# MatthewZhang473/Efficient-Gaussian-Process-on-Graphs

Measured on AMD Instinct MI355X. Metric: GRF kernel-matrices/sec (N=100k graph, m=128 walks; + achieved HBM GB/s of the Gram kernel), higher is better.
Workload: dtype fp64 walk loads, fp32 Phi, exact-product int64 fixed-point Gram, fp32 K

## Files before the change

efficient-gaussian-process-on-graphs_amd/csrc/grf_gram.hip:

```cpp
#include <stdio.h>
#include <stdlib.h>

#include <algorithm>

#include "grf_block.h"

namespace grf {

typedef float f32x4 __attribute__((ext_vector_type(4)));
typedef uint32_t uint4_v __attribute__((ext_vector_type(4)));

#ifndef GRF_GRAM_K_NT
#define GRF_GRAM_K_NT 1
#endif
#if GRF_GRAM_K_NT
#define GRF_K_STORE(v, p) __builtin_nontemporal_store((v), (p))
#define GRF_K_LOAD(p) __builtin_nontemporal_load(p)
#else
#define GRF_K_STORE(v, p) (*(p) = (v))
#define GRF_K_LOAD(p) (*(p))
#endif
#ifndef GRF_GRAM_PIPE_ABLATE
#define GRF_GRAM_PIPE_ABLATE 0
#endif

constexpr int kChunk = 1024;
constexpr int kSub = 8;
constexpr int kPairBytesG = 12;
constexpr int kTripleBytesG = 16;
constexpr int wave_state_bytes(int halves) { return kChunk + halves * 64 * 8; }

__device__ inline long long fx_round(double x) {
    const double magic = 6755399441055744.0;
    const unsigned long long b = (unsigned long long)__double_as_longlong(x + magic);
    const uint32_t hi = (uint32_t)(b >> 32) - 0x43380000u, lo = (uint32_t)b;
    return (long long)(((unsigned long long)hi << 32) | lo);
}

__device__ inline long long fx_fma_round(double a, double v) {
    const double magic = 6755399441055744.0;
    const unsigned long long b = (unsigned long long)__double_as_longlong(__builtin_fma(a, v, magic));
    const uint32_t hi = (uint32_t)(b >> 32) - 0x43380000u, lo = (uint32_t)b;
    return (long long)(((unsigned long long)hi << 32) | lo);
}


__device__ inline int wave_incl_max(int v) {
    v = max(v, __builtin_amdgcn_update_dpp(0, v, 0x111, 0xf, 0xf, false));
    v = max(v, __builtin_amdgcn_update_dpp(0, v, 0x112, 0xf, 0xf, false));
    v = max(v, __builtin_amdgcn_update_dpp(0, v, 0x114, 0xf, 0xf, false));
    v = max(v, __builtin_amdgcn_update_dpp(0, v, 0x118, 0xf, 0xf, false));
    v = max(v, __builtin_amdgcn_update_dpp(0, v, 0x142, 0xa, 0xf, false));
    v = max(v, __builtin_amdgcn_update_dpp(0, v, 0x143, 0xc, 0xf, false));
    return v;
}

template <int NW>
__device__ inline int gram_propagate_ids(unsigned char *bid, int carry, int lane) {
    static_assert(NW == 1 || NW == 2 || NW == 4, "one 4-, 8- or 16-byte LDS access per lane");
    uint32_t w[NW];
    if constexpr (NW == 1) {
        w[0] = reinterpret_cast<uint32_t *>(bid)[lane];
    } else if constexpr (NW == 2) {
        const uint2 x = reinterpret_cast<uint2 *>(bid)[lane];
        w[0] = x.x;
        w[1] = x.y;
    } else {
        const uint4 x = reinterpret_cast<uint4 *>(bid)[lane];
        w[0] = x.x;
        w[1] = x.y;
        w[2] = x.z;
        w[3] = x.w;
    }
    int run = 0;
#pragma unroll
    for (int i = 0; i < NW; ++i) {
        uint32_t o = 0;
#pragma unroll
        for (int b = 0; b < 4; ++b) {
            run = max(run, (int)((w[i] >> (8 * b)) & 0xffu));
            o |= (uint32_t)run << (8 * b);
        }
        w[i] = o;
    }
    int before = __builtin_amdgcn_update_dpp(0, wave_incl_max(run), 0x138, 0xf, 0xf, false);
    before = max(before, carry);
#pragma unroll
    for (int i = 0; i < NW; ++i) {
// ... 37 lines not shown

template <int NW, int TAIL, int kRec>
__device__ __forceinline__ void gram_windows(const GramStream &g, int32_t w0, int32_t c0, int32_t cend, int lane) {
    static_assert(TAIL == 0 || TAIL == 1, "only the last window of a group is ever masked");
    static_assert(kRec == kPairBytesG || kRec == kTripleBytesG, "record pairs or triples");
    const bool last_ok = !TAIL || w0 + (NW - 1) * 64 + lane < cend;
    int m[NW];
#pragma unroll
    for (int u = 0; u < NW; ++u) {
        const int32_t p = w0 + u * 64 + lane;
        m[u] = (u != NW - 1 || last_ok) ? (int)g.st.bid[p - c0] - 1 : 0;
    }
    int32_t pos[NW];
    double sc[NW];
#pragma unroll
    for (int u = 0; u < NW; ++u) {
        pos[u] = g.st.tbase[m[u]] + kRec * (w0 + u * 64 + lane);
        sc[u] = (double)g.st.aval[m[u]] * g.S;
    }
    if (TAIL) {
        pos[NW - 1] = last_ok ? pos[NW - 1] : g.safe;
        sc[NW - 1] = last_ok ? sc[NW - 1] : 0.0;
    }
    __builtin_amdgcn_sched_barrier(0);
    if constexpr (kRec == kTripleBytesG) {
        uint4_v rec[NW];
#pragma unroll
        for (int u = 0; u < NW; ++u) rec[u] = __builtin_amdgcn_raw_buffer_load_b128(g.rec, (uint32_t)pos[u], 0, 0);
        __builtin_amdgcn_sched_barrier(0);
#pragma unroll
        for (int u = 0; u < NW; ++u) {
            const uint32_t cols = rec[u][0], base = cols & 0xe00u;
            uint32_t c[3] = {(cols & 0xfffu) << 3, (base + ((cols >> 12) & 0x3ffu)) << 3, (base + (cols >> 22)) << 3};
#pragma unroll
            for (int q = 0; q < 3; ++q) {
                if (TAIL && u == NW - 1) c[q] = last_ok ? c[q] : (uint32_t)(lane & 15) * 8u;
                const long long v = fx_fma_round(sc[u], (double)__uint_as_float(rec[u][1 + q]));
                __hip_atomic_fetch_add(reinterpret_cast<unsigned long long *>(g.acc + c[q]), (unsigned long long)v,
                                       __ATOMIC_RELAXED, __HIP_MEMORY_SCOPE_WORKGROUP);
            }
        }
        return;
    }
    RecPair rec[NW];
#pragma unroll
    for (int u = 0; u < NW; ++u) {
        const auto v = __builtin_amdgcn_raw_buffer_load_b96(g.rec, (uint32_t)pos[u], 0, 0);
        rec[u].cols = v[0];
        rec[u].v0 = __uint_as_float(v[1]);
        rec[u].v1 = __uint_as_float(v[2]);
    }
    __builtin_amdgcn_sched_barrier(0);
#pragma unroll
    for (int u = 0; u < NW; ++u) {
        const long long q0 = fx_fma_round(sc[u], (double)rec[u].v0);
        const long long q1 = fx_fma_round(sc[u], (double)rec[u].v1);
        uint32_t c0 = rec[u].cols & 0xffffu, c1 = rec[u].cols >> 16;
        if (TAIL && u == NW - 1) {
            c0 = last_ok ? c0 : (uint32_t)(lane & 15) * 8u;
            c1 = last_ok ? c1 : (uint32_t)(lane & 15) * 8u;
        }
        __hip_atomic_fetch_add(reinterpret_cast<unsigned long long *>(g.acc + c0), (unsigned long long)q0,
                               __ATOMIC_RELAXED, __HIP_MEMORY_SCOPE_WORKGROUP);
        __hip_atomic_fetch_add(reinterpret_cast<unsigned long long *>(g.acc + c1), (unsigned long long)q1,
                               __ATOMIC_RELAXED, __HIP_MEMORY_SCOPE_WORKGROUP);
    }
}

__device__ inline float fx_to_float(unsigned long long a, int sh) {
    const int lo = (int)(unsigned)(a & 0xffffffffull);
    const int hi = (int)(a >> 32) - (lo >> 31);
    return ldexpf(fmaf((float)hi, 4294967296.0f, (float)lo), -sh);
}

__device__ __forceinline__ void slot_buckets(uint2 d, int32_t sb, int32_t ovf_base, int32_t *t0, int32_t *cnt) {
    const int32_t inl = min((int32_t)d.x, 2);
    t0[0] = sb + 8;
    cnt[0] = inl;
    t0[1] = ovf_base + kPairBytesG * (int32_t)d.y;
    cnt[1] = (int32_t)d.x - inl;
}

constexpr int kGramUnroll = 8;

template <int kV, int kRec = kPairBytesG>
__device__ __forceinline__ void gram_stream_batch(const GramStream &gs, const int32_t *cnt, const int32_t *t0,
                                                  const float *av, int lane) {
    const GramWaveState &st = gs.st;
    int32_t excl[kV];
    int32_t total = 0;
#pragma unroll
    for (int h = 0; h < kV; ++h) {
        const int32_t inc = wave_inclusive_scan<int32_t>(cnt[h]) + total;
        excl[h] = inc - cnt[h];
        total = __builtin_amdgcn_readlane(inc, 63);
    }
#pragma unroll
    for (int h = 0; h < kV; ++h) {
        st.tbase[h * 64 + lane] = t0[h] - kRec * excl[h];
        st.aval[h * 64 + lane] = av[h];
    }
    int carry = 0;
    const int32_t chunk = total <= 256 ? 256 : total <= 512 ? 512 : kChunk;
    for (int32_t c0 = 0; c0 < total; c0 += chunk) {
        const int32_t cend = (total - c0) < chunk ? total : c0 + chunk;
        if (chunk == 256) reinterpret_cast<uint32_t *>(st.bid)[lane] = 0u;
        else if (chunk == 512) reinterpret_cast<uint2 *>(st.bid)[lane] = make_uint2(0u, 0u);
        else reinterpret_cast<uint4 *>(st.bid)[lane] = make_uint4(0u, 0u, 0u, 0u);
        __builtin_amdgcn_wave_barrier();
#pragma unroll
        for (int h = 0; h < kV; ++h)
            if (cnt[h] > 0 && excl[h] >= c0 && excl[h] < cend)
                st.bid[excl[h] - c0] = (unsigned char)(h * 64 + lane + 1);
        __builtin_amdgcn_wave_barrier();
        carry = chunk == 256   ? gram_propagate_ids<1>(st.bid, carry, lane)
                : chunk == 512 ? gram_propagate_ids<2>(st.bid, carry, lane)
                               : gram_propagate_ids<4>(st.bid, carry, lane);
        __builtin_amdgcn_wave_barrier();
        int32_t w0 = c0;
        for (; w0 + 64 * kGramUnroll <= cend; w0 += 64 * kGramUnroll)
            gram_windows<kGramUnroll, 0, kRec>(gs, w0, c0, cend, lane);
        if (w0 < cend) {
            static_assert(kGramUnroll == 8, "the tail switch lists 1 .. 8 windows");
            switch ((cend - w0 + 63) >> 6) {
                case 1: gram_windows<1, 1, kRec>(gs, w0, c0, cend, lane); break;
                case 2: gram_windows<2, 1, kRec>(gs, w0, c0, cend, lane); break;
                case 3: gram_windows<3, 1, kRec>(gs, w0, c0, cend, lane); break;
                case 4: gram_windows<4, 1, kRec>(gs, w0, c0, cend, lane); break;
                case 5: gram_windows<5, 1, kRec>(gs, w0, c0, cend, lane); break;
                case 6: gram_windows<6, 1, kRec>(gs, w0, c0, cend, lane); break;
                case 7: gram_windows<7, 1, kRec>(gs, w0, c0, cend, lane); break;
                default: gram_windows<8, 1, kRec>(gs, w0, c0, cend, lane); break;
            }
        }
        __builtin_amdgcn_wave_barrier();
    }
}

typedef unsigned long long u64x2 __attribute__((ext_vector_type(2)));

template <bool kZero>
__device__ __forceinline__ void gram_tile_out(unsigned long long *acc, float *krow, bool vec, int64_t c_lo,
                                              int64_t wlen, int sh, bool addk, int tid, int threads) {
#if GRF_GRAM_PIPE_ABLATE == 2
    constexpr bool store = !kZero;
#else
    constexpr bool store = true;
#endif
    u64x2 *acc2 = reinterpret_cast<u64x2 *>(acc);
    const u64x2 z2 = {0ull, 0ull};
    int64_t done = c_lo;
    if (vec) {
        const int64_t n4 = wlen / 4;
        f32x4 *k4 = reinterpret_cast<f32x4 *>(krow);
        for (int64_t i = c_lo / 4 + tid; i < n4; i += threads) {
            const u64x2 a = acc2[2 * i], b = acc2[2 * i + 1];
            f32x4 o;
            o[0] = fx_to_float(a[0], sh);
            o[1] = fx_to_float(a[1], sh);
            o[2] = fx_to_float(b[0], sh);
            o[3] = fx_to_float(b[1], sh);
            if (addk) o += __builtin_nontemporal_load(&k4[i]);
            if (store) GRF_K_STORE(o, &k4[i]);
            if (kZero) {
                acc2[2 * i] = z2;
                acc2[2 * i + 1] = z2;
            }
        }
        done = n4 * 4;
    }
    for (int64_t i = done + tid; i < wlen; i += threads) {
        if (store) krow[i] = addk ? fx_to_float(acc[i], sh) + krow[i] : fx_to_float(acc[i], sh);
        if (kZero) acc[i] = 0ull;
    }
}

constexpr size_t gram_lds_bytes(int64_t W, int waves, int halves) {
    return (size_t)W * 8 + (size_t)waves * wave_state_bytes(halves);
}

struct GramTiles {
    int64_t rows, W, nb;
    bool sym;
    int32_t k_begin, k_end;
    int64_t J_off = 0;
    int64_t t_rows = -1;
    bool add_k = false;
    __host__ __device__ int64_t count(int64_t J) const {
        if (!sym) return rows;
        const int64_t c = (J + 1) * W;
        return c < rows ? c : rows;
    }
    __host__ __device__ int64_t before(int64_t J) const {
        if (!sym) return J * rows;
        const int64_t full = (rows + W - 1) / W - 1;
        return J <= full ? W * J * (J + 1) / 2 : W * full * (full + 1) / 2 + (J - full) * rows;
    }
    __host__ __device__ int64_t total() const { return before(nb); }
    __device__ void locate(int64_t t, int64_t &J, int64_t &r) const {
        if (!sym) {
            J = t / rows;
        } else {
            J = (int64_t)((sqrt(8.0 * (double)(t / W) + 1.0) - 1.0) * 0.5);
            if (J > nb - 1) J = nb - 1;
            while (J > 0 && before(J) > t) --J;
            while (J < nb - 1 && before(J + 1) <= t) ++J;
        }
        r = t - before(J);
    }
};

template <int kWaves, int kHalves, bool kSlot, int kRec>
__global__ __launch_bounds__(64 * kWaves) void gram_sparse_kernel(
    int64_t n_total, int64_t row_begin, GramTiles tl, int64_t t_begin, const int64_t *__restrict__ ptr,
    const int32_t *__restrict__ idx, const float *__restrict__ val, const uint2 *__restrict__ t_desc,
    const unsigned char *__restrict__ t_rec, int32_t unit, const int32_t *__restrict__ rowshift,
    float *__restrict__ K, int64_t ldk, const uint16_t *__restrict__ t_split,
    int64_t ovf_base, int32_t balance, const int32_t *__restrict__ row_cuts) {
    extern __shared__ __attribute__((aligned(16))) unsigned long long acc[];
    static_assert(!kSlot || kHalves == 1, "slot streams: 2 virtual buckets per nonzero, u8 ids <= 128");
    static_assert(!kSlot || kRec == kPairBytesG, "slots hold pairs");
    const int tid = threadIdx.x, lane = tid & 63, wave = tid >> 6;
    const int64_t W = tl.W;
    constexpr int kB = 64 * kHalves;
    constexpr int kV = kSlot ? 2 * kHalves : kHalves;

    int64_t J, r;
    tl.locate(t_begin + (int64_t)blockIdx.x, J, r);
    const int64_t J_local = J;
    J += tl.J_off;
    const int64_t row = row_begin + r;
    const int64_t j0 = J * W;
    const int64_t t_rows = tl.t_rows < 0 ? n_total : tl.t_rows;
    const int64_t wlen = (t_rows - j0) < W ? (t_rows - j0) : W;
    const int64_t e0 = ptr[row], e1 = ptr[row + 1];
    const int64_t boff = J * n_total;
    const int sh = rowshift[row];
    const int32_t line0 = kSlot ? 0 : (int32_t)t_desc[boff].x;
    const unsigned char *brec = t_rec + (int64_t)line0 * unit;
    const int dsub = (t_split && tl.sym && r >= J_local * W) ? (int)(((r - J_local * W) * kSub) / W) : 0;

    u64x2 *acc2 = reinterpret_cast<u64x2 *>(acc);
    const u64x2 z2 = {0ull, 0ull};
    for (int64_t i = tid; i < W / 2; i += 64 * kWaves) acc2[i] = z2;
    if (kWaves > 1) __syncthreads();
    else __builtin_amdgcn_wave_barrier();

    const GramStream gs{gram_wave_state(acc, W, wave, kV),
                        __builtin_amdgcn_make_buffer_rsrc(const_cast<unsigned char *>(brec), (short)0, 0x7fffffff,
                                                          0x00020000),
                        reinterpret_cast<unsigned char *>(acc), ldexp(1.0, sh), kSlot ? 8 : 0};
    const int64_t nnz_row = e1 - e0, share = (nnz_row + kWaves - 1) / kWaves;
    int64_t ws0 = balance ? e0 + (wave * share < nnz_row ? wave * share : nnz_row) : e0 + (int64_t)wave * kB;
    int64_t ws1 = balance ? e0 + ((wave + 1) * share < nnz_row ? (wave + 1) * share : nnz_row) : e1;
    if (row_cuts) {
        static_assert(8 % kWaves == 0, "row cuts: 8 shares per row");
        constexpr int kStep = 8 / kWaves;
        ws0 = e0 + row_cuts[row * 8 + wave * kStep];
        ws1 = wave + 1 < kWaves ? e0 + row_cuts[row * 8 + (wave + 1) * kStep] : e1;
    }
    const int64_t gstep = (balance || row_cuts) ? kB : (int64_t)kB * kWaves;
    for (int64_t g0 = ws0; g0 < ws1; g0 += gstep) {
        const int64_t gend = (balance || row_cuts) ? ((g0 + kB) < ws1 ? g0 + kB : ws1) : e1;
        int32_t cnt[kV], t0[kV];
        float av[kV];
#pragma unroll
        for (int h = 0; h < kHalves; ++h) {
            const int64_t e = g0 + h * 64 + lane;
            int32_t k = e < gend ? idx[e] : -1;
            if (k < tl.k_begin || k >= tl.k_end) k = -1;
            const float a = k >= 0 ? val[e] : 0.f;
            if constexpr (kSlot) {
                const int64_t sb = 32 * (boff + (k >= 0 ? k : 0));
                const uint2 d = k >= 0 ? *reinterpret_cast<const uint2 *>(t_rec + sb) : make_uint2(0u, 0u);
                slot_buckets(d, (int32_t)sb, (int32_t)ovf_base, &t0[2 * h], &cnt[2 * h]);
                av[2 * h] = a;
                av[2 * h + 1] = a;
            } else {
                av[h] = a;
                const uint2 d = k >= 0 ? t_desc[boff + k] : make_uint2((uint32_t)line0, 0u);
                const int32_t skip = (dsub > 0 && k >= 0) ? min((int32_t)(t_split[(boff + k) * kSub + dsub] >> 1), (int32_t)d.y) : 0;
                t0[h] = ((int32_t)d.x - line0) * unit + kRec * skip;
                cnt[h] = (int32_t)d.y - skip;
            }
        }
        gram_stream_batch<kV, kRec>(gs, cnt, t0, av, lane);
    }
    if (kWaves > 1) __syncthreads();
    else __builtin_amdgcn_wave_barrier();

    gram_tile_out<false>(acc, K + r * ldk + j0, (ldk & 3) == 0 && (j0 & 3) == 0, (int64_t)dsub * (W / kSub), wlen, sh,
                         tl.add_k, tid, 64 * kWaves);
}

__device__ __forceinline__ void pipe_barrier() { asm volatile("s_waitcnt lgkmcnt(0)\n\ts_barrier" ::: "memory"); }

struct PipeNz {
    int32_t k;
    float a;
    int32_t sh;
    int32_t nb;
    int64_t ws0;
};

template <int kWv>
__global__ __launch_bounds__(64 * kWv) void gram_slot_pipe_kernel(
    int64_t n_cols, int64_t row_begin, int64_t rows, int64_t W, int64_t t_rows, int64_t n_tiles,
    const int64_t *__restrict__ ptr, const int32_t *__restrict__ idx, const float *__restrict__ val,
    const unsigned char *__restrict__ t_rec, const int32_t *__restrict__ rowshift, float *__restrict__ K,
    int64_t ldk, int64_t ovf_base, int64_t pad_cap, const int32_t *__restrict__ pad_cnt) {
    extern __shared__ __attribute__((aligned(16))) unsigned long long acc[];
    const int tid = threadIdx.x, lane = tid & 63, wave = tid >> 6;
    const int64_t G = gridDim.x;
    const int64_t n_mine = (int64_t)blockIdx.x < n_tiles ? (n_tiles - 1 - (int64_t)blockIdx.x) / G + 1 : 0;
    u64x2 *acc2 = reinterpret_cast<u64x2 *>(acc);
    const u64x2 z2 = {0ull, 0ull};
    for (int64_t q = tid; q < W / 2; q += 64 * kWv) acc2[q] = z2;
    const GramWaveState wst = gram_wave_state(acc, W, wave, 2);
    const __amdgpu_buffer_rsrc_t rec_rs =
        __builtin_amdgcn_make_buffer_rsrc(const_cast<unsigned char *>(t_rec), (short)0, 0x7fffffff, 0x00020000);
    auto tile_row = [&](int64_t i, int64_t &J) -> int64_t {
        const int64_t t = (int64_t)blockIdx.x + i * G;
        J = t / rows;
        return row_begin + (t - J * rows);
    };
    auto load_bounds = [&](int64_t i, int64_t &pv, int32_t &pc, int32_t &shv) {
        if (i >= n_mine) {
            pv = 0;
            pc = 0;
            shv = 0;
            return;
        }
        int64_t J;
        const int64_t row = tile_row(i, J);
        if (pad_cap > 0) {
            const __amdgpu_buffer_rsrc_t rc =
                __builtin_amdgcn_make_buffer_rsrc(const_cast<int32_t *>(pad_cnt + row), (short)0, 4, 0x00020000);
            pc = (int32_t)__builtin_amdgcn_raw_buffer_load_b32(rc, 0u, 0, 0);
        } else {
            const __amdgpu_buffer_rsrc_t rp =
                __builtin_amdgcn_make_buffer_rsrc(const_cast<int64_t *>(ptr + row), (short)0, 16, 0x00020000);
            const auto v = __builtin_amdgcn_raw_buffer_load_b64(rp, (uint32_t)(lane & 1) * 8u, 0, 0);
            pv = (int64_t)(((uint64_t)v[1] << 32) | v[0]);
        }
        const __amdgpu_buffer_rsrc_t rs =
            __builtin_amdgcn_make_buffer_rsrc(const_cast<int32_t *>(rowshift + row), (short)0, 4, 0x00020000);
        shv = (int32_t)__builtin_amdgcn_raw_buffer_load_b32(rs, 0u, 0, 0);
    };
    auto load_nz = [&](int64_t i, int64_t pv, int32_t pc, int32_t shv, PipeNz &z) {
        if (i >= n_mine) {
            z = PipeNz{-1, 0.f, 0, 0, 0};
            return;
        }
        auto lane_i64 = [&](int l) {
            const uint32_t lo = (uint32_t)__builtin_amdgcn_readlane((int)(uint32_t)pv, l);
            const uint32_t hi = (uint32_t)__builtin_amdgcn_readlane((int)(uint32_t)((uint64_t)pv >> 32), l);
            return (int64_t)(((uint64_t)hi << 32) | lo);
        };
        int64_t e0, e1;
        if (pad_cap > 0) {
            int64_t J;
            e0 = tile_row(i, J) * pad_cap;
            e1 = e0 + (int64_t)__builtin_amdgcn_readlane(pc, 0);
        } else {
            e0 = lane_i64(0);
            e1 = lane_i64(1);
        }
        const int64_t nnz = e1 - e0, share = (nnz + kWv - 1) / kWv;
        const int64_t s0 = wave * share < nnz ? wave * share : nnz, s1 = (wave + 1) * share < nnz ? (wave + 1) * share : nnz;
        const int64_t e = e0 + s0 + lane;
        const bool ok = s0 + lane < s1;
        z.k = ok ? idx[e] : -1;
        z.a = ok ? val[e] : 0.f;
        z.sh = shv;
        z.nb = (int32_t)(s1 - s0);
        z.ws0 = e0 + s0;
    };
    auto load_hdr = [&](int64_t i, int32_t k) -> uint2 {
        if (i >= n_mine || k < 0) return make_uint2(0u, 0u);
        int64_t J;
        tile_row(i, J);
        return *reinterpret_cast<const uint2 *>(t_rec + 32 * (J * n_cols + k));
    };
    auto run_batch = [&](const GramStream &gs, int64_t J, int32_t k, float a, uint2 d) {
        int32_t cnt[2], t0[2];
        const float av[2] = {a, a};
        slot_buckets(d, (int32_t)(32 * (J * n_cols + (k >= 0 ? k : 0))), (int32_t)ovf_base, t0, cnt);
        gram_stream_batch<2>(gs, cnt, t0, av, lane);
    };
    int64_t pv = 0;
    int32_t pc = 0, shv;
    PipeNz T0, T1;
    load_bounds(0, pv, pc, shv);
    load_nz(0, pv, pc, shv, T0);
    uint2 d0 = load_hdr(0, T0.k);
    load_bounds(1, pv, pc, shv);
    load_nz(1, pv, pc, shv, T1);
    load_bounds(2, pv, pc, shv);
    __builtin_amdgcn_s_waitcnt(0);
    pipe_barrier();
    for (int64_t i = 0; i < n_mine; ++i) {
        const uint2 d1 = load_hdr(i + 1, T1.k);
        PipeNz T2;
        load_nz(i + 2, pv, pc, shv, T2);
        load_bounds(i + 3, pv, pc, shv);
        int64_t J;
        const int64_t row = tile_row(i, J);
        if (GRF_GRAM_PIPE_ABLATE != 1) {
            const GramStream gs{wst, rec_rs, reinterpret_cast<unsigned char *>(acc), ldexp(1.0, T0.sh), 8};
            run_batch(gs, J, T0.k, T0.a, d0);
            for (int32_t g = 64; g < T0.nb; g += 64) {
                const int64_t e = T0.ws0 + g + lane;
                const bool ok = g + lane < T0.nb;
                const int32_t k = ok ? idx[e] : -1;
                const float a = ok ? val[e] : 0.f;
                const uint2 d = k >= 0 ? *reinterpret_cast<const uint2 *>(t_rec + 32 * (J * n_cols + k)) : make_uint2(0u, 0u);
                run_batch(gs, J, k, a, d);
            }
        }
        __builtin_amdgcn_s_waitcnt(0);
        pipe_barrier();
        const int64_t r = row - row_begin, j0 = J * W;
        const int64_t wlen = (t_rows - j0) < W ? (t_rows - j0) : W;
        gram_tile_out<true>(acc, K + r * ldk + j0, (ldk & 3) == 0 && (j0 & 3) == 0, 0, wlen, T0.sh, false, tid,
                            64 * kWv);
        pipe_barrier();
        T0 = T1;
        d0 = d1;
        T1 = T2;
    }
}

__global__ __launch_bounds__(256) void hub_panel_kernel(int64_t n_rows, const int64_t *__restrict__ ptr,
                                                        const int32_t *__restrict__ idx, const float *__restrict__ val,
                                                        const int32_t *__restrict__ hub_pos, float *__restrict__ P,
                                                        int64_t ldp) {
    const int64_t row = (int64_t)blockIdx.x * 4 + (threadIdx.x >> 6);
    if (row >= n_rows) return;
    const int lane = threadIdx.x & 63;
    const int64_t e1 = ptr[row + 1];
    for (int64_t e = ptr[row] + lane; e < e1; e += 64) {
        const int32_t q = hub_pos[idx[e]];
        if (q >= 0) P[row * ldp + q] = val[e];
    }
}

__global__ __launch_bounds__(256) void transpose_drop_kernel(int64_t n_bands, int64_t n_cols, uint2 *__restrict__ t_desc,
                                                             const int32_t *__restrict__ cols, int32_t n_drop) {
    const int64_t t = (int64_t)blockIdx.x * 256 + threadIdx.x;
    if (t >= n_bands * n_drop) return;
    const int64_t J = t / n_drop;
    t_desc[J * n_cols + cols[t - J * n_drop]].y = 0u;
}

__device__ __forceinline__ void gram_mirror_tri_coords(int64_t nt, int64_t b, int64_t &bi_out, int64_t &bj_out) {
    int64_t bi = (int64_t)(((double)(2 * nt + 1) - sqrt((double)(2 * nt + 1) * (double)(2 * nt + 1) - 8.0 * (double)b)) * 0.5);
    auto first = [nt](int64_t i) { return i * nt - i * (i - 1) / 2; };
    if (bi < 0) bi = 0;
    if (bi > nt - 1) bi = nt - 1;
    while (bi > 0 && first(bi) > b) --bi;
    while (bi < nt - 1 && first(bi + 1) <= b) ++bi;
    bi_out = bi;
    bj_out = bi + (b - first(bi));
}

__device__ __forceinline__ void gram_mirror_block_at(int64_t n, int64_t bi, int64_t bj, float *__restrict__ K,
                                                     int64_t ldk, float (*tile)[65]) {
    const int64_t i0 = bi * 64, j0 = bj * 64;
    const int t = threadIdx.x;
    const bool full = i0 + 64 <= n && j0 + 64 <= n && (ldk & 3) == 0;
#pragma unroll
    for (int q = 0; q < 4; ++q) {
        const int y = (t >> 4) + 16 * q, x = (t & 15) * 4;
        const int64_t i = i0 + y;
        if (full) {
            const f32x4 v = __builtin_nontemporal_load(reinterpret_cast<const f32x4 *>(K + i * ldk + j0 + x));
            tile[y][x] = v[0]; tile[y][x + 1] = v[1]; tile[y][x + 2] = v[2]; tile[y][x + 3] = v[3];
        } else {
#pragma unroll
            for (int c = 0; c < 4; ++c) tile[y][x + c] = (i < n && j0 + x + c < n) ? K[i * ldk + j0 + x + c] : 0.f;
        }
    }
    __syncthreads();
#pragma unroll
    for (int q = 0; q < 4; ++q) {
        const int y = (t >> 4) + 16 * q, x = (t & 15) * 4;
        const int64_t j = j0 + y;
        if (full && bi != bj) {
            f32x4 v;
            v[0] = tile[x][y]; v[1] = tile[x + 1][y]; v[2] = tile[x + 2][y]; v[3] = tile[x + 3][y];
            __builtin_nontemporal_store(v, reinterpret_cast<f32x4 *>(K + j * ldk + i0 + x));
        } else {
#pragma unroll
            for (int c = 0; c < 4; ++c) {
                const int64_t i = i0 + x + c;
                if (j < n && i < n && j > i) K[j * ldk + i] = tile[x + c][y];
            }
        }
    }
}

__device__ __forceinline__ void gram_mirror_block_swz_at(int64_t n, int64_t bi, int64_t bj, float *__restrict__ K,
                                                         int64_t ldk, float *__restrict__ tile) {
    const int64_t i0 = bi * 64, j0 = bj * 64;
    const int t = threadIdx.x;
    const bool full = i0 + 64 <= n && j0 + 64 <= n && (ldk & 3) == 0 && bi != bj;
    if (!full) {
// ... 71 lines not shown
}

}

using namespace grf;

extern "C" {
#pragma GCC visibility push(default)

size_t grf_gram_workspace_bytes(void) { return 256; }

struct GramArgs {
    int64_t n_total;
    int64_t row_begin;
    const int64_t *ptr;
    const int32_t *idx;
    const float *val;
    int64_t pad_cap;
    const int32_t *pad_cnt;
    int32_t unit;
    int32_t rec_kind;
    const uint32_t *t_desc;
    const void *t_rec;
    const void *t_split;
    const int32_t *rowshift;
    const int32_t *row_cuts;
    float *K;
    int64_t ldk;
    hipStream_t st;
};

static int32_t gram_check(const char *fn, bool args_ok, int32_t unit, const void *t_rec, int64_t ldk, int64_t ld_min,
                          int64_t band_width) {
    GRF_REQUIRE(args_ok, GRF_EINVAL, "%s: bad arguments", fn);
    GRF_REQUIRE(unit == GRF_REC_LINE || unit == GRF_REC_PACKED || unit == GRF_REC_SLOT, GRF_EINVAL,
                "%s: rec_unit must be GRF_REC_LINE, GRF_REC_PACKED or GRF_REC_SLOT", fn);
    GRF_REQUIRE(((uintptr_t)t_rec & 127) == 0, GRF_EINVAL, "%s: t_rec must be 128-byte aligned", fn);
    GRF_REQUIRE(ldk >= ld_min, GRF_EINVAL, "%s: ldk < %lld columns", fn, (long long)ld_min);
    GRF_REQUIRE(band_width >= 64 && band_width % 64 == 0 && band_width <= 8192, GRF_EUNSUPPORTED,
                "%s: band_width must be a multiple of 64 in [64, 8192]", fn);
    return GRF_OK;
}

static int32_t gram_tiles_launch(const GramArgs &a, const GramTiles &tl, int64_t t_first, int64_t t_last) {
    const bool slot = a.unit == GRF_REC_SLOT;
    GRF_REQUIRE(a.rec_kind == GRF_REC_PAIRS ||
                    (a.rec_kind == GRF_REC_TRIPLES && a.unit == GRF_REC_LINE && tl.W <= 4096 && !a.t_split),
                GRF_EINVAL, "gram: GRF_REC_TRIPLES needs line buckets, band_width <= 4096 and no t_split");
    const unsigned char *rec = reinterpret_cast<const unsigned char *>(a.t_rec);
    const int64_t ovf_base = slot ? 32 * tl.nb * a.n_total : 0;
    if (slot) {
        GRF_REQUIRE(!a.t_split, GRF_EUNSUPPORTED, "gram: GRF_REC_SLOT has no split variant");
        GRF_REQUIRE(ovf_base < ((int64_t)1 << 30), GRF_EUNSUPPORTED,
                    "gram: GRF_REC_SLOT slots beyond 32-bit record offsets");
        const bool pipe = [] {
            const char *e = getenv("GRF_GRAM_PIPE");
            return !e || atoi(e) != 0;
        }();
        const bool pipe_ok = !tl.sym && tl.t_rows >= 0 && !tl.add_k && tl.k_begin == 0 &&
                             tl.k_end == (int32_t)a.n_total && t_first == 0 && t_last == tl.total() && tl.J_off == 0;
        GRF_REQUIRE(a.pad_cap == 0 || pipe_ok, GRF_EUNSUPPORTED,
                    "gram: padded rows need the pipelined column-block kernel (a whole non-symmetric launch)");
        if ((pipe || a.pad_cap > 0) && pipe_ok) {
            const size_t lds = gram_lds_bytes(tl.W, 8, 2);
            int dev = 0, n_cu = 0;
            GRF_CHECK_HIP(hipGetDevice(&dev));
            GRF_CHECK_HIP(hipDeviceGetAttribute(&n_cu, hipDeviceAttributeMultiprocessorCount, dev));
            const int per_cu = (int)std::max<int64_t>(1, (int64_t)(160 * 1024) / (int64_t)lds);
            const int64_t grid = std::min<int64_t>((int64_t)std::max(n_cu, 1) * per_cu, t_last);
            gram_slot_pipe_kernel<8><<<(unsigned)grid, 512, lds, a.st>>>(
                a.n_total, a.row_begin, tl.rows, tl.W, tl.t_rows, t_last, a.ptr, a.idx, a.val, rec, a.rowshift, a.K,
                a.ldk, ovf_base, a.pad_cap, a.pad_cnt);
            GRF_CHECK_LAUNCH("gram_slot_pipe_kernel");
            return GRF_OK;
        }
    }
    const uint16_t *split = tl.sym ? (const uint16_t *)a.t_split : nullptr;
    const int waves = (slot || tl.W > 4096) ? 8 : 4;
    const size_t lds = gram_lds_bytes(tl.W, waves, (slot || waves == 4) ? 2 : 1);
    const int32_t balance = (slot || tl.t_rows < 0) ? 1 : 0;
    const int64_t max_tiles = ((1ll << 32) - 1) / (64 * waves);
    for (int64_t t0 = t_first; t0 < t_last; t0 += max_tiles) {
        const int64_t nt = (t_last - t0) < max_tiles ? (t_last - t0) : max_tiles;
#define GRF_GRAM_LAUNCH(WV, H, SLOT, REC)                                                                         \
    gram_sparse_kernel<WV, H, SLOT, REC><<<(unsigned)nt, 64 * WV, lds, a.st>>>(                                   \
        a.n_total, a.row_begin, tl, t0, a.ptr, a.idx, a.val, reinterpret_cast<const uint2 *>(a.t_desc), rec, a.unit, \
        a.rowshift, a.K, a.ldk, split, ovf_base, balance, a.row_cuts)
        if (slot) GRF_GRAM_LAUNCH(8, 1, true, kPairBytesG);
        else if (waves == 8) GRF_GRAM_LAUNCH(8, 1, false, kPairBytesG);
        else if (a.rec_kind == GRF_REC_TRIPLES) GRF_GRAM_LAUNCH(4, 2, false, kTripleBytesG);
        else GRF_GRAM_LAUNCH(4, 2, false, kPairBytesG);
#undef GRF_GRAM_LAUNCH
        GRF_CHECK_LAUNCH("gram_sparse_kernel");
    }
    return GRF_OK;
}

static int32_t gram_sparse_rows_impl(const char *fn, int32_t rec_kind, int64_t n_total, int64_t row_begin, int64_t row_end,
                                     int64_t k_begin, int64_t k_end, const int64_t *ptr, const int32_t *idx,
                                     const float *val, int64_t band_width, int32_t rec_unit, const uint32_t *t_desc,
                                     const void *t_rec, const int32_t *t_rowshift, float *K, int64_t ldk,
                                     grf_stream_t stream) {
    int32_t rc = gram_check(fn,
                            n_total >= 0 && 0 <= row_begin && row_begin <= row_end && row_end <= n_total && ptr &&
                                t_desc && K && t_rowshift && t_rec,
                            rec_unit, t_rec, ldk, n_total, band_width);
    if (rc != GRF_OK) return rc;
    GRF_REQUIRE(0 <= k_begin && k_begin <= k_end && k_end <= n_total, GRF_EINVAL, "%s: bad column slice [%lld, %lld)",
                fn, (long long)k_begin, (long long)k_end);
    if (row_end == row_begin || n_total == 0) return GRF_OK;
    const GramTiles tl{row_end - row_begin, band_width, cdiv<int64_t>(n_total, band_width), false, (int32_t)k_begin,
                       (int32_t)k_end};
    const GramArgs a{n_total,  row_begin, ptr,    idx,   val,     0,          nullptr,
                     rec_unit, rec_kind,  t_desc, t_rec, nullptr, t_rowshift, nullptr, K, ldk, S(stream)};
    return gram_tiles_launch(a, tl, 0, tl.total());
}

int32_t grf_gram_sparse(int64_t n_total, int64_t row_begin, int64_t row_end, const int64_t *ptr, const int32_t *idx,
                        const float *val, int64_t band_width, int32_t rec_unit, const uint32_t *t_desc,
                        const void *t_rec, const int32_t *t_rowshift, float *K, int64_t ldk, void *workspace,
                        size_t workspace_bytes, grf_stream_t stream) {
    return gram_sparse_rows_impl("grf_gram_sparse", GRF_REC_PAIRS, n_total, row_begin, row_end, 0, n_total, ptr, idx, val,
                                 band_width, rec_unit, t_desc, t_rec, t_rowshift, K, ldk, stream);
}

int32_t grf_gram_sparse_rec(int32_t rec_kind, int64_t n_total, int64_t row_begin, int64_t row_end, const int64_t *ptr,
                            const int32_t *idx, const float *val, int64_t band_width, int32_t rec_unit,
                            const uint32_t *t_desc, const void *t_rec, const int32_t *t_rowshift, float *K, int64_t ldk,
                            grf_stream_t stream) {
    return gram_sparse_rows_impl("grf_gram_sparse_rec", rec_kind, n_total, row_begin, row_end, 0, n_total, ptr, idx, val,
                                 band_width, rec_unit, t_desc, t_rec, t_rowshift, K, ldk, stream);
}

static int32_t gram_sparse_upper_impl(const char *fn, int32_t rec_kind, int64_t n_total, const int64_t *ptr, const int32_t *idx,
                                      const float *val, int64_t band_width, int32_t rec_unit, const uint32_t *t_desc,
                                      const void *t_rec, const void *t_split, const int32_t *t_rowshift,
                                      const int32_t *row_cuts, float *K, int64_t ldk, int32_t part_begin,
                                      int32_t part_end, int32_t n_parts, bool add_k, grf_stream_t stream) {
    int32_t rc = gram_check(fn, n_total >= 0 && ptr && t_desc && K && t_rowshift && t_rec, rec_unit, t_rec, ldk,
                            n_total, band_width);
    if (rc != GRF_OK) return rc;
    GRF_REQUIRE(n_parts >= 1 && 0 <= part_begin && part_begin <= part_end && part_end <= n_parts, GRF_EINVAL,
                "%s: bad tile parts [%d, %d) of %d", fn, part_begin, part_end, n_parts);
    if (n_total == 0 || part_begin == part_end) return GRF_OK;
    GramTiles tl{n_total, band_width, cdiv<int64_t>(n_total, band_width), true, 0, (int32_t)n_total};
    tl.add_k = add_k;
    const int64_t total = tl.total();
    const int64_t t0 = total * part_begin / n_parts, t1 = total * part_end / n_parts;
    if (t1 <= t0) return GRF_OK;
    GRF_REQUIRE(!row_cuts || rec_unit != GRF_REC_SLOT, GRF_EUNSUPPORTED, "%s: row cuts with slot buckets", fn);
    const GramArgs a{n_total,  0,        ptr,    idx,   val,     0,          nullptr,
                     rec_unit, rec_kind, t_desc, t_rec, t_split, t_rowshift, row_cuts, K, ldk, S(stream)};
    return gram_tiles_launch(a, tl, t0, t1);
}

int32_t grf_gram_sparse_sym(int64_t n_total, const int64_t *ptr, const int32_t *idx, const float *val,
                            int64_t band_width, int32_t rec_unit, const uint32_t *t_desc, const void *t_rec,
                            const void *t_split, const int32_t *t_rowshift, float *K, int64_t ldk, void *workspace, size_t workspace_bytes,
                            grf_stream_t stream) {
    int32_t rc = gram_sparse_upper_impl("grf_gram_sparse_sym", GRF_REC_PAIRS, n_total, ptr, idx, val, band_width, rec_unit, t_desc,
                                        t_rec, t_split, t_rowshift, nullptr, K, ldk, 0, 1, 1, false, stream);
    if (rc != GRF_OK || n_total == 0) return rc;
    return grf_gram_mirror(n_total, K, ldk, 0, stream);
}

int32_t grf_gram_sparse_upper_ex(int64_t n_total, const int64_t *ptr, const int32_t *idx, const float *val,
                                 int64_t band_width, int32_t rec_unit, const uint32_t *t_desc, const void *t_rec,
                                 const void *t_split, const int32_t *t_rowshift, const int32_t *row_cuts, float *K,
                                 int64_t ldk, int32_t part_begin, int32_t part_end, int32_t n_parts, int32_t add_k,
                                 grf_stream_t stream) {
    return gram_sparse_upper_impl("grf_gram_sparse_upper_ex", GRF_REC_PAIRS, n_total, ptr, idx, val, band_width, rec_unit, t_desc,
                                  t_rec, t_split, t_rowshift, row_cuts, K, ldk, part_begin, part_end, n_parts,
                                  add_k != 0, stream);
}
// ... 222 lines not shown
```

Measured before the change: 45.73.

## Add specialised plain symmetric Gram tile path with 32-bit tile indexing

Adds a specialised kernel path for the common full symmetric Gram case without splits, row cuts or accumulate. It locates tiles with 32-bit reciprocal division and a float sqrt, splits each row's nonzeros evenly across waves, and prefetches the next batch of bucket descriptors during streaming. It uses a smaller window unroll of 4 and 32-bit loop indices in the tile output, aiming to cut integer and address overhead and register pressure. It adds a second kernel instantiation, and the float-sqrt locate depends on its correction step to stay exact.

```diff
diff --git a/efficient-gaussian-process-on-graphs_amd/csrc/grf_gram.hip b/efficient-gaussian-process-on-graphs_amd/csrc/grf_gram.hip
--- a/efficient-gaussian-process-on-graphs_amd/csrc/grf_gram.hip
+++ b/efficient-gaussian-process-on-graphs_amd/csrc/grf_gram.hip
@@ -4,6 +4,7 @@
 #include <algorithm>
 
 #include "grf_block.h"
+#include "grf_gram_tiles.h"
 
 namespace grf {
 
@@ -207,8 +208,21 @@
 }
 
 constexpr int kGramUnroll = 8;
-
-template <int kV, int kRec = kPairBytesG>
+constexpr int kPlainUnroll = 4;
+
+template <int N, int kRec>
+__device__ __forceinline__ void gram_tail_group(const GramStream &gs, int nw, int32_t w0, int32_t c0, int32_t cend,
+                                                int lane) {
+    if constexpr (N > 1) {
+        if (nw < N) {
+            gram_tail_group<N - 1, kRec>(gs, nw, w0, c0, cend, lane);
+            return;
+        }
+    }
+    gram_windows<N, 1, kRec>(gs, w0, c0, cend, lane);
+}
+
+template <int kV, int kRec = kPairBytesG, int kU = kGramUnroll>
 __device__ __forceinline__ void gram_stream_batch(const GramStream &gs, const int32_t *cnt, const int32_t *t0,
                                                   const float *av, int lane) {
     const GramWaveState &st = gs.st;
@@ -243,21 +257,9 @@
                                : gram_propagate_ids<4>(st.bid, carry, lane);
         __builtin_amdgcn_wave_barrier();
         int32_t w0 = c0;
-        for (; w0 + 64 * kGramUnroll <= cend; w0 += 64 * kGramUnroll)
-            gram_windows<kGramUnroll, 0, kRec>(gs, w0, c0, cend, lane);
-        if (w0 < cend) {
-            static_assert(kGramUnroll == 8, "the tail switch lists 1 .. 8 windows");
-            switch ((cend - w0 + 63) >> 6) {
-                case 1: gram_windows<1, 1, kRec>(gs, w0, c0, cend, lane); break;
-                case 2: gram_windows<2, 1, kRec>(gs, w0, c0, cend, lane); break;
-                case 3: gram_windows<3, 1, kRec>(gs, w0, c0, cend, lane); break;
-                case 4: gram_windows<4, 1, kRec>(gs, w0, c0, cend, lane); break;
-                case 5: gram_windows<5, 1, kRec>(gs, w0, c0, cend, lane); break;
-                case 6: gram_windows<6, 1, kRec>(gs, w0, c0, cend, lane); break;
-                case 7: gram_windows<7, 1, kRec>(gs, w0, c0, cend, lane); break;
-                default: gram_windows<8, 1, kRec>(gs, w0, c0, cend, lane); break;
-            }
-        }
+        for (; w0 + 64 * kU <= cend; w0 += 64 * kU)
+            gram_windows<kU, 0, kRec>(gs, w0, c0, cend, lane);
+        if (w0 < cend) gram_tail_group<kU, kRec>(gs, (cend - w0 + 63) >> 6, w0, c0, cend, lane);
         __builtin_amdgcn_wave_barrier();
     }
 }
@@ -265,8 +267,8 @@
 typedef unsigned long long u64x2 __attribute__((ext_vector_type(2)));
 
 template <bool kZero>
-__device__ __forceinline__ void gram_tile_out(unsigned long long *acc, float *krow, bool vec, int64_t c_lo,
-                                              int64_t wlen, int sh, bool addk, int tid, int threads) {
+__device__ __forceinline__ void gram_tile_out(unsigned long long *acc, float *krow, bool vec, int32_t c_lo,
+                                              int32_t wlen, int sh, bool addk, int tid, int threads) {
 #if GRF_GRAM_PIPE_ABLATE == 2
     constexpr bool store = !kZero;
 #else
@@ -274,11 +276,11 @@
 #endif
     u64x2 *acc2 = reinterpret_cast<u64x2 *>(acc);
     const u64x2 z2 = {0ull, 0ull};
-    int64_t done = c_lo;
+    int32_t done = c_lo;
     if (vec) {
-        const int64_t n4 = wlen / 4;
+        const int32_t n4 = wlen / 4;
         f32x4 *k4 = reinterpret_cast<f32x4 *>(krow);
-        for (int64_t i = c_lo / 4 + tid; i < n4; i += threads) {
+        for (int32_t i = c_lo / 4 + tid; i < n4; i += threads) {
             const u64x2 a = acc2[2 * i], b = acc2[2 * i + 1];
             f32x4 o;
             o[0] = fx_to_float(a[0], sh);
@@ -294,7 +296,7 @@
         }
         done = n4 * 4;
     }
-    for (int64_t i = done + tid; i < wlen; i += threads) {
+    for (int32_t i = done + tid; i < wlen; i += threads) {
         if (store) krow[i] = addk ? fx_to_float(acc[i], sh) + krow[i] : fx_to_float(acc[i], sh);
         if (kZero) acc[i] = 0ull;
     }
@@ -304,40 +306,75 @@
     return (size_t)W * 8 + (size_t)waves * wave_state_bytes(halves);
 }
 
-struct GramTiles {
-    int64_t rows, W, nb;
-    bool sym;
-    int32_t k_begin, k_end;
-    int64_t J_off = 0;
-    int64_t t_rows = -1;
-    bool add_k = false;
-    __host__ __device__ int64_t count(int64_t J) const {
-        if (!sym) return rows;
-        const int64_t c = (J + 1) * W;
-        return c < rows ? c : rows;
-    }
-    __host__ __device__ int64_t before(int64_t J) const {
-        if (!sym) return J * rows;
-        const int64_t full = (rows + W - 1) / W - 1;
-        return J <= full ? W * J * (J + 1) / 2 : W * full * (full + 1) / 2 + (J - full) * rows;
-    }
-    __host__ __device__ int64_t total() const { return before(nb); }
-    __device__ void locate(int64_t t, int64_t &J, int64_t &r) const {
-        if (!sym) {
-            J = t / rows;
-        } else {
-            J = (int64_t)((sqrt(8.0 * (double)(t / W) + 1.0) - 1.0) * 0.5);
-            if (J > nb - 1) J = nb - 1;
-            while (J > 0 && before(J) > t) --J;
-            while (J < nb - 1 && before(J + 1) <= t) ++J;
-        }
-        r = t - before(J);
-    }
-};
-
-template <int kWaves, int kHalves, bool kSlot, int kRec>
+__device__ __forceinline__ void pipe_barrier() { asm volatile("s_waitcnt lgkmcnt(0)\n\ts_barrier" ::: "memory"); }
+
+template <int kWaves, int kHalves, int kRec>
+__device__ __forceinline__ void gram_plain_tile(unsigned long long *acc, uint32_t n_total, const GramTiles32 &t32,
+                                                uint32_t t, const int64_t *__restrict__ ptr,
+                                                const int32_t *__restrict__ idx, const float *__restrict__ val,
+                                                const uint2 *__restrict__ t_desc,
+                                                const unsigned char *__restrict__ t_rec, int32_t unit,
+                                                const int32_t *__restrict__ rowshift, float *__restrict__ K,
+                                                int64_t ldk) {
+    static_assert(kWaves > 1, "the plain tile synchronises its waves with s_barrier");
+    const int tid = threadIdx.x, lane = tid & 63, wave = __builtin_amdgcn_readfirstlane(tid >> 6);
+    constexpr int kB = 64 * kHalves;
+    uint32_t J, r;
+    t32.locate(t, J, r);
+    J += t32.J_off;
+    const uint32_t W = t32.W, j0 = J * W;
+    const int32_t wlen = (int32_t)((n_total - j0) < W ? (n_total - j0) : W);
+    const uint2 *bdesc = t_desc + (uint64_t)J * n_total;
+    const int64_t e0 = ptr[r], e1 = ptr[r + 1];
+    const int sh = rowshift[r];
+    const int32_t line0 = (int32_t)bdesc[0].x;
+    const int32_t *ridx = idx + e0;
+    const float *rval = val + e0;
+    const int32_t nnz_row = (int32_t)(e1 - e0), share = (nnz_row + kWaves - 1) / kWaves;
+    const int32_t s0 = min(wave * share, nnz_row), s1 = min((wave + 1) * share, nnz_row);
+
+    int32_t k[kHalves];
+    float av[kHalves];
+    uint2 d[kHalves];
+    auto load_batch = [&](int32_t g) {
+        const int32_t gend = min(g + kB, s1);
+#pragma unroll
+        for (int h = 0; h < kHalves; ++h) {
+            const int32_t e = g + h * 64 + lane;
+            k[h] = e < gend ? ridx[e] : -1;
+            av[h] = e < gend ? rval[e] : 0.f;
+        }
+#pragma unroll
+        for (int h = 0; h < kHalves; ++h) d[h] = k[h] >= 0 ? bdesc[k[h]] : make_uint2((uint32_t)line0, 0u);
+    };
+    load_batch(s0);
+    u64x2 *acc2 = reinterpret_cast<u64x2 *>(acc);
+    const u64x2 z2 = {0ull, 0ull};
+    for (int32_t i = tid; i < (int32_t)(W / 2); i += 64 * kWaves) acc2[i] = z2;
+    const GramStream gs{gram_wave_state(acc, W, wave, kHalves),
+                        __builtin_amdgcn_make_buffer_rsrc(const_cast<unsigned char *>(t_rec + (int64_t)line0 * unit),
+                                                          (short)0, 0x7fffffff, 0x00020000),
+                        reinterpret_cast<unsigned char *>(acc), ldexp(1.0, sh), 0};
+    pipe_barrier();
+    for (int32_t g = s0; g < s1;) {
+        int32_t cnt[kHalves], t0[kHalves];
+#pragma unroll
+        for (int h = 0; h < kHalves; ++h) {
+            t0[h] = ((int32_t)d[h].x - line0) * unit;
+            cnt[h] = (int32_t)d[h].y;
+        }
+        gram_stream_batch<kHalves, kRec, kPlainUnroll>(gs, cnt, t0, av, lane);
+        g += kB;
+        if (g < s1) load_batch(g);
+    }
+    __syncthreads();
+    gram_tile_out<false>(acc, K + (int64_t)r * ldk + j0, (ldk & 3) == 0 && (j0 & 3) == 0, 0, wlen, sh, false, tid,
+                         64 * kWaves);
+}
+
+template <int kWaves, int kHalves, bool kSlot, int kRec, bool kPlain = false>
 __global__ __launch_bounds__(64 * kWaves) void gram_sparse_kernel(
-    int64_t n_total, int64_t row_begin, GramTiles tl, int64_t t_begin, const int64_t *__restrict__ ptr,
+    int64_t n_total, int64_t row_begin, GramTiles tl, GramTiles32 t32, int64_t t_begin, const int64_t *__restrict__ ptr,
     const int32_t *__restrict__ idx, const float *__restrict__ val, const uint2 *__restrict__ t_desc,
     const unsigned char *__restrict__ t_rec, int32_t unit, const int32_t *__restrict__ rowshift,
     float *__restrict__ K, int64_t ldk, const uint16_t *__restrict__ t_split,
@@ -345,6 +382,12 @@
     extern __shared__ __attribute__((aligned(16))) unsigned long long acc[];
     static_assert(!kSlot || kHalves == 1, "slot streams: 2 virtual buckets per nonzero, u8 ids <= 128");
     static_assert(!kSlot || kRec == kPairBytesG, "slots hold pairs");
+    if constexpr (kPlain) {
+        static_assert(!kSlot, "the plain tile reads line or packed buckets");
+        gram_plain_tile<kWaves, kHalves, kRec>(acc, (uint32_t)n_total, t32, (uint32_t)t_begin + blockIdx.x, ptr, idx, val,
+                                               t_desc, t_rec, unit, rowshift, K, ldk);
+        return;
+    }
     const int tid = threadIdx.x, lane = tid & 63, wave = tid >> 6;
     const int64_t W = tl.W;
     constexpr int kB = 64 * kHalves;
@@ -367,7 +410,7 @@
 
     u64x2 *acc2 = reinterpret_cast<u64x2 *>(acc);
     const u64x2 z2 = {0ull, 0ull};
-    for (int64_t i = tid; i < W / 2; i += 64 * kWaves) acc2[i] = z2;
+    for (int32_t i = tid; i < (int32_t)(W / 2); i += 64 * kWaves) acc2[i] = z2;
     if (kWaves > 1) __syncthreads();
     else __builtin_amdgcn_wave_barrier();
 
@@ -414,11 +457,9 @@
     if (kWaves > 1) __syncthreads();
     else __builtin_amdgcn_wave_barrier();
 
-    gram_tile_out<false>(acc, K + r * ldk + j0, (ldk & 3) == 0 && (j0 & 3) == 0, (int64_t)dsub * (W / kSub), wlen, sh,
+    gram_tile_out<false>(acc, K + r * ldk + j0, (ldk & 3) == 0 && (j0 & 3) == 0, dsub * (int32_t)(W / kSub), (int32_t)wlen, sh,
                          tl.add_k, tid, 64 * kWaves);
 }
-
-__device__ __forceinline__ void pipe_barrier() { asm volatile("s_waitcnt lgkmcnt(0)\n\ts_barrier" ::: "memory"); }
 
 struct PipeNz {
     int32_t k;
@@ -547,7 +588,7 @@
         pipe_barrier();
         const int64_t r = row - row_begin, j0 = J * W;
         const int64_t wlen = (t_rows - j0) < W ? (t_rows - j0) : W;
-        gram_tile_out<true>(acc, K + r * ldk + j0, (ldk & 3) == 0 && (j0 & 3) == 0, 0, wlen, T0.sh, false, tid,
+        gram_tile_out<true>(acc, K + r * ldk + j0, (ldk & 3) == 0 && (j0 & 3) == 0, 0, (int32_t)wlen, T0.sh, false, tid,
                             64 * kWv);
         pipe_barrier();
         T0 = T1;
@@ -785,14 +826,20 @@
     const int64_t max_tiles = ((1ll << 32) - 1) / (64 * waves);
     for (int64_t t0 = t_first; t0 < t_last; t0 += max_tiles) {
         const int64_t nt = (t_last - t0) < max_tiles ? (t_last - t0) : max_tiles;
-#define GRF_GRAM_LAUNCH(WV, H, SLOT, REC)                                                                         \
-    gram_sparse_kernel<WV, H, SLOT, REC><<<(unsigned)nt, 64 * WV, lds, a.st>>>(                                   \
-        a.n_total, a.row_begin, tl, t0, a.ptr, a.idx, a.val, reinterpret_cast<const uint2 *>(a.t_desc), rec, a.unit, \
-        a.rowshift, a.K, a.ldk, split, ovf_base, balance, a.row_cuts)
-        if (slot) GRF_GRAM_LAUNCH(8, 1, true, kPairBytesG);
-        else if (waves == 8) GRF_GRAM_LAUNCH(8, 1, false, kPairBytesG);
-        else if (a.rec_kind == GRF_REC_TRIPLES) GRF_GRAM_LAUNCH(4, 2, false, kTripleBytesG);
-        else GRF_GRAM_LAUNCH(4, 2, false, kPairBytesG);
+        GramTiles32 t32{};
+        const bool plain = !slot && waves == 4 && tl.sym && tl.t_rows < 0 && a.row_begin == 0 && !split &&
+                           !a.row_cuts && !tl.add_k && tl.k_begin == 0 && tl.k_end == a.n_total &&
+                           tl.rows == a.n_total && gram_tiles32(tl, a.n_total, t0, t0 + nt, t32);
+#define GRF_GRAM_LAUNCH(WV, H, SLOT, REC, PLAIN)                                                                  \
+    gram_sparse_kernel<WV, H, SLOT, REC, PLAIN><<<(unsigned)nt, 64 * WV, lds, a.st>>>(                            \
+        a.n_total, a.row_begin, tl, t32, t0, a.ptr, a.idx, a.val, reinterpret_cast<const uint2 *>(a.t_desc), rec, \
+        a.unit, a.rowshift, a.K, a.ldk, split, ovf_base, balance, a.row_cuts)
+        if (slot) GRF_GRAM_LAUNCH(8, 1, true, kPairBytesG, false);
+        else if (waves == 8) GRF_GRAM_LAUNCH(8, 1, false, kPairBytesG, false);
+        else if (a.rec_kind == GRF_REC_TRIPLES && plain) GRF_GRAM_LAUNCH(4, 2, false, kTripleBytesG, true);
+        else if (a.rec_kind == GRF_REC_TRIPLES) GRF_GRAM_LAUNCH(4, 2, false, kTripleBytesG, false);
+        else if (plain) GRF_GRAM_LAUNCH(4, 2, false, kPairBytesG, true);
+        else GRF_GRAM_LAUNCH(4, 2, false, kPairBytesG, false);
 #undef GRF_GRAM_LAUNCH
         GRF_CHECK_LAUNCH("gram_sparse_kernel");
     }
diff --git a/efficient-gaussian-process-on-graphs_amd/csrc/grf_gram_tiles.h b/efficient-gaussian-process-on-graphs_amd/csrc/grf_gram_tiles.h
--- /dev/null
+++ b/efficient-gaussian-process-on-graphs_amd/csrc/grf_gram_tiles.h
@@ -0,0 +1,109 @@
+#pragma once
+#include <math.h>
+#include <stdint.h>
+
+#if defined(__HIPCC__) || defined(__CUDACC__)
+#define GRF_TILES_HD __host__ __device__
+#else
+#define GRF_TILES_HD
+#endif
+
+namespace grf {
+
+struct GramTiles {
+    int64_t rows, W, nb;
+    bool sym;
+    int32_t k_begin, k_end;
+    int64_t J_off = 0;
+    int64_t t_rows = -1;
+    bool add_k = false;
+    GRF_TILES_HD int64_t count(int64_t J) const {
+        if (!sym) return rows;
+        const int64_t c = (J + 1) * W;
+        return c < rows ? c : rows;
+    }
+    GRF_TILES_HD int64_t before(int64_t J) const {
+        if (!sym) return J * rows;
+        const int64_t full = (rows + W - 1) / W - 1;
+        return J <= full ? W * J * (J + 1) / 2 : W * full * (full + 1) / 2 + (J - full) * rows;
+    }
+    GRF_TILES_HD int64_t total() const { return before(nb); }
+    GRF_TILES_HD void locate(int64_t t, int64_t &J, int64_t &r) const {
+        if (!sym) {
+            J = t / rows;
+        } else {
+            J = (int64_t)((sqrt(8.0 * (double)(t / W) + 1.0) - 1.0) * 0.5);
+            if (J > nb - 1) J = nb - 1;
+            while (J > 0 && before(J) > t) --J;
+            while (J < nb - 1 && before(J + 1) <= t) ++J;
+        }
+        r = t - before(J);
+    }
+};
+
+struct GramRecip {
+    uint32_t mul, sh;
+    GRF_TILES_HD uint32_t div(uint32_t x) const { return (uint32_t)(((uint64_t)x * mul) >> sh); }
+};
+
+inline GramRecip gram_recip(uint32_t d) {
+    uint32_t l = 0;
+    while (((uint64_t)1 << l) < d) ++l;
+    return {(uint32_t)((((uint64_t)1 << (31 + l)) / d) + 1), 31 + l};
+}
+
+struct GramTiles32 {
+    uint32_t rows, W;
+    uint32_t full;
+    uint32_t tri_end;
+    GramRecip rW, rR;
+    uint32_t J_off;
+
+    GRF_TILES_HD void locate_est(uint32_t t, float s, uint32_t &J, uint32_t &r) const {
+        if (t >= tri_end) {
+            const uint32_t u = t - tri_end, q = rR.div(u);
+            J = full + q;
+            r = u - q * rows;
+            return;
+        }
+        const uint32_t q = rW.div(t);
+        int32_t j = (int32_t)((s - 1.0f) * 0.5f);
+        if (j < 0) j = 0;
+        uint32_t b = (uint32_t)j;
+        if (b * (b + 1) / 2 > q) --b;
+        else if ((b + 1) * (b + 2) / 2 <= q) ++b;
+        J = b;
+        r = t - W * (b * (b + 1) / 2);
+    }
+    GRF_TILES_HD static float root_arg(uint32_t q) { return (float)(8u * q + 1u); }
+    GRF_TILES_HD void locate(uint32_t t, uint32_t &J, uint32_t &r) const {
+        float s = 0.f;
+        if (t < tri_end) {
+#if defined(__HIP_DEVICE_COMPILE__)
+            s = __builtin_amdgcn_sqrtf(root_arg(rW.div(t)));
+#else
+            s = sqrtf(root_arg(rW.div(t)));
+#endif
+        }
+        locate_est(t, s, J, r);
+    }
+};
+
+inline bool gram_tiles32(const GramTiles &tl, int64_t n_total, int64_t t_first, int64_t t_last, GramTiles32 &o) {
+    const int64_t lim = (int64_t)1 << 31;
+    if (t_last <= t_first || t_last - 1 >= lim || n_total >= lim || tl.rows >= lim || tl.rows < 1 || tl.W < 64 ||
+        tl.W >= lim || tl.J_off < 0 || tl.J_off + tl.nb >= lim)
+        return false;
+    const int64_t full = tl.sym ? (tl.rows + tl.W - 1) / tl.W - 1 : 0;
+    const int64_t tri_end = tl.sym ? tl.before(full < tl.nb ? full : tl.nb) : 0;
+    o.rows = (uint32_t)tl.rows;
+    o.W = (uint32_t)tl.W;
+    o.full = (uint32_t)(full < tl.nb ? full : tl.nb);
+    o.tri_end = (uint32_t)(tri_end < lim ? tri_end : lim);
+    o.rW = gram_recip(o.W);
+    o.rR = gram_recip(o.rows);
+    o.J_off = (uint32_t)tl.J_off;
+    return true;
+}
+
+}
```

After: 47.42, median of 6. 3.7% higher.
